# pearsonlab/autoencoded-vocal-analysis

Measured on AMD Instinct MI355X. Metric: spectrograms/sec, VAE train step (fwd+bwd+Adam), 128x128, batch 256 per GPU, higher is better.
Workload: dtype f32 (fc1/fc8 products, the forward convolutions with >= 8 input channels and the fused backward kernels (data gradient AND weight gradient): fp32 operands as three bf16 limbs on bf16 MFMA, six limb products, fp32 accumulate; the 1<->8-channel layers, convt6's forward, conv7's forward and the small f; 1 GPU; configs[1]: mouse_sylls VAE, batch 256 synthetic 128x128 fp32 spectrograms per GPU, z=32, train step = zero_grad+forward+backward+Adam, device-resident batches; global_batch=256, per_gpu_batch=256, z_dim=32, parallelism=dp1

## Files before the change

autoencoded-vocal-analysis_amd/csrc/conv_recomp.h:

```cpp
#pragma once
#include "conv_common.h"
#include "conv_mfma.h"

template <int C>
struct Conv1to8Core {
  static constexpr int NG = (C + 15) / 16;
  static constexpr int XCP = 16 * NG + 2;
  static constexpr int XS_F = 8 * XCP;
  static constexpr int XE = 7 * (C + 2);
  static constexpr int NLX = (XE + 63) / 64;
  static constexpr int NUW = NG + (NG + 3) / 4;
  static constexpr int LDS_FLOATS = 4 * XS_F;
  static_assert(NLX <= 16 && NUW <= 16, "masks are 16 bits wide");
  float xr[NLX];
  float wA[3];
  unsigned xin;
  int lane, wave;

  __device__ __forceinline__ void init(const float* __restrict__ G1, float* __restrict__ xs_all, int tid) {
    lane = tid & 63; wave = tid >> 6;
    const int m = lane & 15, kgA = lane >> 4, half = m >> 3, co = m & 7, ky = kgA - half;
#pragma unroll
    for (int c = 0; c < 3; ++c) {
      float v = (ky >= 0 && ky <= 2) ? G1[(ky * 3 + c) * 8 + co] : 0.f;
      asm volatile("" : "+v"(v));
      wA[c] = v;
    }
    float* xs = xs_all + wave * XS_F;
    for (int e = lane; e < XS_F; e += 64) xs[e] = 0.f;
    xin = 0u;
  }
  __device__ __forceinline__ int win_row(int pr) const { return pr < 4 ? 2 * wave + pr : 4 + pr; }

  __device__ __forceinline__ void load(const float* __restrict__ src, int b, int H, int W, int gy0, int gx0) {
    const float* __restrict__ base = src + (size_t)b * H * W;
    xin = 0u;
#pragma unroll
    for (int i = 0; i < NLX; ++i) {
      const int e = lane + 64 * i, pr = e / (C + 2), pc = e - pr * (C + 2);
      const int gy = gy0 - 1 + win_row(pr), gx = gx0 - 1 + pc;
      const bool ok = e < XE && gy >= 0 && gy < H && gx >= 0 && gx < W;
      const int cy = min(max(gy, 0), H - 1), cx = min(max(gx, 0), W - 1);
      xr[i] = base[cy * W + cx];
      xin |= ok ? (1u << i) : 0u;
    }
  }
  template <class PRO>
  __device__ __forceinline__ void stage(float* __restrict__ xs_all, PRO pro) {
    float* __restrict__ xs = xs_all + wave * XS_F;
#pragma unroll
    for (int i = 0; i < NLX; ++i) {
      const int e = lane + 64 * i, pr = e / (C + 2), pc = e - pr * (C + 2);
      if (e < XE) xs[pr * XCP + pc] = ((xin >> i) & 1u) ? pro(xr[i]) : 0.f;
    }
    __builtin_amdgcn_fence(__ATOMIC_RELEASE, "wavefront");
    __builtin_amdgcn_wave_barrier();
  }
  __device__ __forceinline__ bool unit(int u, int& row, int& col, int& quad, int& pb, int& g) const {
    const int n = lane & 15, kg = lane >> 4;
    const bool own = u < NG;
    g = own ? u : wave + 4 * (u - NG);
    pb = own ? 0 : 4;
    row = (own ? 2 * wave : 8) + (kg >> 1);
    col = 16 * g + n;
    quad = kg & 1;
    return g < NG && col < C && (own || (kg >> 1) == 0);
  }
  __device__ __forceinline__ f32x4 mma(const float* __restrict__ xs_all, int pb, int g) const {
    const float* __restrict__ xs = xs_all + wave * XS_F;
    const int n = lane & 15, kg = lane >> 4;
    const float* p = xs + (pb + kg) * XCP + 16 * g + n;
    const float b0 = p[0], b1 = p[1], b2 = p[2];
    f32x4 acc = {0.f, 0.f, 0.f, 0.f};
    acc = __builtin_amdgcn_mfma_f32_16x16x4f32(wA[0], b0, acc, 0, 0, 0);
    acc = __builtin_amdgcn_mfma_f32_16x16x4f32(wA[1], b1, acc, 0, 0, 0);
    acc = __builtin_amdgcn_mfma_f32_16x16x4f32(wA[2], b2, acc, 0, 0, 0);
    return acc;
  }
};

template <int C, typename ACT>
struct DU1to8Stager {
  using Core = Conv1to8Core<C>;
  static constexpr int LDS_FLOATS = Core::LDS_FLOATS;
  Core core;
  avaf4 y2[Core::NUW];
  unsigned yin;
  __device__ __forceinline__ void init(const RecompArgs& rc, float* xs_all, int tid = (int)threadIdx.x) {
    core.init(rc.G1, xs_all, tid);
    yin = 0u;
  }
  __device__ __forceinline__ void load(const float* __restrict__ in, const float* __restrict__ in2, int b, int H, int W,
                                       int gy0, int gx0) {
    core.load(in, b, H, W, gy0, gx0);
    const ACT* __restrict__ base2 = ava_as<ACT>(in2) + (size_t)b * H * W * 8;
    yin = 0u;
#pragma unroll
    for (int u = 0; u < Core::NUW; ++u) {
      int row, col, quad, pb, g;
      const bool v = core.unit(u, row, col, quad, pb, g);
      const int gy = gy0 + row, gx = gx0 + col;
      const bool ok = v && gy >= 0 && gy < H && gx >= 0 && gx < W;
      const int cy = min(max(gy, 0), H - 1), cx = min(max(gx, 0), W - 1);
      y2[u] = ava_ld4<ACT>(base2 + (cy * W + cx) * 8 + 4 * quad);
      yin |= ok ? (1u << u) : 0u;
    }
  }
  __device__ __forceinline__ void store(float* __restrict__ lds, const float* __restrict__ coef, float* __restrict__ xs_all) {
    core.stage(xs_all, [](float v) { return v; });
    const float* ca = coef + 4 * ((core.lane >> 4) & 1);
    const avaf4 kA = {ca[0], ca[1], ca[2], ca[3]}, kB = {ca[32], ca[33], ca[34], ca[35]}, kC = {ca[64], ca[65], ca[66], ca[67]};
#pragma unroll
    for (int u = 0; u < Core::NUW; ++u) {
      int row, col, quad, pb, g;
      const bool v = core.unit(u, row, col, quad, pb, g);
      if (u >= Core::NG && core.wave + 4 * (u - Core::NG) >= Core::NG) continue;
      const f32x4 acc = core.mma(xs_all, pb, g);
      const bool in = (yin >> u) & 1u;
      avaf4 o;
#pragma unroll
      for (int r = 0; r < 4; ++r) {
        const float y = y2[u][r];
        const float du = fmaf(kA[r], acc[r], fmaf(kB[r], y, kC[r]));
        o[r] = (in && y > 0.f) ? du : 0.f;
      }
      if (v) *reinterpret_cast<avaf4*>(lds + (row * C + col) * 8 + 4 * quad) = o;
    }
  }

  __device__ __forceinline__ void store_limb(unsigned char* __restrict__ lds, const float* __restrict__ coef, float* __restrict__ xs_all) {
    constexpr int PLANE_BYTES = 9 * C * 16;
    core.stage(xs_all, [](float v) { return v; });
    const float* ca = coef + 4 * ((core.lane >> 4) & 1);
    const avaf4 kA = {ca[0], ca[1], ca[2], ca[3]}, kB = {ca[32], ca[33], ca[34], ca[35]}, kC = {ca[64], ca[65], ca[66], ca[67]};
#pragma unroll
    for (int u = 0; u < Core::NUW; ++u) {
      int row, col, quad, pb, g;
      const bool v = core.unit(u, row, col, quad, pb, g);
      if (u >= Core::NG && core.wave + 4 * (u - Core::NG) >= Core::NG) continue;
      const f32x4 acc = core.mma(xs_all, pb, g);
      const bool in = (yin >> u) & 1u;
      avaf4 o;
#pragma unroll
      for (int r = 0; r < 4; ++r) {
        const float y = y2[u][r];
        const float du = fmaf(kA[r], acc[r], fmaf(kB[r], y, kC[r]));
        o[r] = (in && y > 0.f) ? du : 0.f;
      }
      ava_u32x2 p0, p1, p2;
      uint32_t a, b, c;
      ava_limb_split2(o[0], o[1], a, b, c); p0[0] = a; p1[0] = b; p2[0] = c;
      ava_limb_split2(o[2], o[3], a, b, c); p0[1] = a; p1[1] = b; p2[1] = c;
      unsigned char* d = lds + (row * C + col) * 16 + quad * 8;
      if (v) {
        *reinterpret_cast<ava_u32x2*>(d) = p0;
        *reinterpret_cast<ava_u32x2*>(d + PLANE_BYTES) = p1;
        *reinterpret_cast<ava_u32x2*>(d + 2 * PLANE_BYTES) = p2;
      }
    }
  }
};
```

Measured before the change: 179,700 spectrograms/s.

## Pack tail columns and row-8 share into one mixed MFMA unit per wave

```diff
diff --git a/autoencoded-vocal-analysis_amd/csrc/conv_recomp.h b/autoencoded-vocal-analysis_amd/csrc/conv_recomp.h
--- a/autoencoded-vocal-analysis_amd/csrc/conv_recomp.h
+++ b/autoencoded-vocal-analysis_amd/csrc/conv_recomp.h
@@ -5,13 +5,17 @@
 template <int C>
 struct Conv1to8Core {
   static constexpr int NG = (C + 15) / 16;
+  static constexpr int NGF = C / 16, REM = C - 16 * NGF;
+  static constexpr int RW = (C + 3) / 4;
   static constexpr int XCP = 16 * NG + 2;
   static constexpr int XS_F = 8 * XCP;
-  static constexpr int XE = 7 * (C + 2);
+  static constexpr int XE4 = 4 * (C + 2);
+  static constexpr int XE = XE4 + 3 * (RW + 2);
   static constexpr int NLX = (XE + 63) / 64;
-  static constexpr int NUW = NG + (NG + 3) / 4;
+  static constexpr int NUW = NGF + 1;
   static constexpr int LDS_FLOATS = 4 * XS_F;
   static_assert(NLX <= 16 && NUW <= 16, "masks are 16 bits wide");
+  static_assert(REM + RW <= 16 && 3 * RW + RW + 2 <= XCP, "the mixed unit holds the pair's last columns and this wave's share of row 8");
   float xr[NLX];
   float wA[3];
   unsigned xin;
@@ -30,6 +34,12 @@
     for (int e = lane; e < XS_F; e += 64) xs[e] = 0.f;
     xin = 0u;
   }
+  __device__ __forceinline__ bool elem(int e, int& pr, int& pc) const {
+    if (e < XE4) { pr = e / (C + 2); pc = e - pr * (C + 2); return true; }
+    const int f = e - XE4, r = f / (RW + 2);
+    pr = 4 + r; pc = RW * wave + f - r * (RW + 2);
+    return e < XE && pc < C + 2;
+  }
   __device__ __forceinline__ int win_row(int pr) const { return pr < 4 ? 2 * wave + pr : 4 + pr; }
 
   __device__ __forceinline__ void load(const float* __restrict__ src, int b, int H, int W, int gy0, int gx0) {
@@ -37,9 +47,10 @@
     xin = 0u;
 #pragma unroll
     for (int i = 0; i < NLX; ++i) {
-      const int e = lane + 64 * i, pr = e / (C + 2), pc = e - pr * (C + 2);
+      int pr, pc;
+      const bool ex = elem(lane + 64 * i, pr, pc);
       const int gy = gy0 - 1 + win_row(pr), gx = gx0 - 1 + pc;
-      const bool ok = e < XE && gy >= 0 && gy < H && gx >= 0 && gx < W;
+      const bool ok = ex && (unsigned)gy < (unsigned)H && (unsigned)gx < (unsigned)W;
       const int cy = min(max(gy, 0), H - 1), cx = min(max(gx, 0), W - 1);
       xr[i] = base[cy * W + cx];
       xin |= ok ? (1u << i) : 0u;
@@ -50,26 +61,27 @@
     float* __restrict__ xs = xs_all + wave * XS_F;
 #pragma unroll
     for (int i = 0; i < NLX; ++i) {
-      const int e = lane + 64 * i, pr = e / (C + 2), pc = e - pr * (C + 2);
-      if (e < XE) xs[pr * XCP + pc] = ((xin >> i) & 1u) ? pro(xr[i]) : 0.f;
+      int pr, pc;
+      if (elem(lane + 64 * i, pr, pc)) xs[pr * XCP + pc] = ((xin >> i) & 1u) ? pro(xr[i]) : 0.f;
     }
     __builtin_amdgcn_fence(__ATOMIC_RELEASE, "wavefront");
     __builtin_amdgcn_wave_barrier();
   }
-  __device__ __forceinline__ bool unit(int u, int& row, int& col, int& quad, int& pb, int& g) const {
-    const int n = lane & 15, kg = lane >> 4;
-    const bool own = u < NG;
-    g = own ? u : wave + 4 * (u - NG);
+  __device__ __forceinline__ bool unit(int u, int& row, int& col, int& quad, int& pb) const {
+    const int n = lane & 15, kg = lane >> 4, half = kg >> 1;
+    quad = kg & 1;
+    if (u < NGF) { row = 2 * wave + half; col = 16 * u + n; pb = 0; return true; }
+    const bool own = n < REM;
+    const int c8 = RW * wave + n - REM;
+    row = own ? 2 * wave + half : 8;
+    col = own ? 16 * NGF + n : min(c8, C - 1);
     pb = own ? 0 : 4;
-    row = (own ? 2 * wave : 8) + (kg >> 1);
-    col = 16 * g + n;
-    quad = kg & 1;
-    return g < NG && col < C && (own || (kg >> 1) == 0);
+    return own || (n < REM + RW && c8 < C && half == 0);
   }
-  __device__ __forceinline__ f32x4 mma(const float* __restrict__ xs_all, int pb, int g) const {
+  __device__ __forceinline__ f32x4 mma(const float* __restrict__ xs_all, int pb, int col) const {
     const float* __restrict__ xs = xs_all + wave * XS_F;
-    const int n = lane & 15, kg = lane >> 4;
-    const float* p = xs + (pb + kg) * XCP + 16 * g + n;
+    const int kg = lane >> 4;
+    const float* p = xs + (pb + kg) * XCP + col;
     const float b0 = p[0], b1 = p[1], b2 = p[2];
     f32x4 acc = {0.f, 0.f, 0.f, 0.f};
     acc = __builtin_amdgcn_mfma_f32_16x16x4f32(wA[0], b0, acc, 0, 0, 0);
@@ -97,10 +109,10 @@
     yin = 0u;
 #pragma unroll
     for (int u = 0; u < Core::NUW; ++u) {
-      int row, col, quad, pb, g;
-      const bool v = core.unit(u, row, col, quad, pb, g);
+      int row, col, quad, pb;
+      const bool v = core.unit(u, row, col, quad, pb);
       const int gy = gy0 + row, gx = gx0 + col;
-      const bool ok = v && gy >= 0 && gy < H && gx >= 0 && gx < W;
+      const bool ok = v && (unsigned)gy < (unsigned)H && (unsigned)gx < (unsigned)W;
       const int cy = min(max(gy, 0), H - 1), cx = min(max(gx, 0), W - 1);
       y2[u] = ava_ld4<ACT>(base2 + (cy * W + cx) * 8 + 4 * quad);
       yin |= ok ? (1u << u) : 0u;
@@ -112,10 +124,9 @@
     const avaf4 kA = {ca[0], ca[1], ca[2], ca[3]}, kB = {ca[32], ca[33], ca[34], ca[35]}, kC = {ca[64], ca[65], ca[66], ca[67]};
 #pragma unroll
     for (int u = 0; u < Core::NUW; ++u) {
-      int row, col, quad, pb, g;
-      const bool v = core.unit(u, row, col, quad, pb, g);
-      if (u >= Core::NG && core.wave + 4 * (u - Core::NG) >= Core::NG) continue;
-      const f32x4 acc = core.mma(xs_all, pb, g);
+      int row, col, quad, pb;
+      const bool v = core.unit(u, row, col, quad, pb);
+      const f32x4 acc = core.mma(xs_all, pb, col);
       const bool in = (yin >> u) & 1u;
       avaf4 o;
 #pragma unroll
@@ -135,10 +146,9 @@
     const avaf4 kA = {ca[0], ca[1], ca[2], ca[3]}, kB = {ca[32], ca[33], ca[34], ca[35]}, kC = {ca[64], ca[65], ca[66], ca[67]};
 #pragma unroll
     for (int u = 0; u < Core::NUW; ++u) {
-      int row, col, quad, pb, g;
-      const bool v = core.unit(u, row, col, quad, pb, g);
-      if (u >= Core::NG && core.wave + 4 * (u - Core::NG) >= Core::NG) continue;
-      const f32x4 acc = core.mma(xs_all, pb, g);
+      int row, col, quad, pb;
+      const bool v = core.unit(u, row, col, quad, pb);
+      const f32x4 acc = core.mma(xs_all, pb, col);
       const bool in = (yin >> u) & 1u;
       avaf4 o;
 #pragma unroll
```

After: 181,100 spectrograms/s (median of 6 runs). About the same (+0.8%).
